# quinlan-lab/STRling

Measured on AMD Instinct MI355X. Metric: reads/sec through extract+cluster, 30x 150 bp WGS; 1/2/4/8 MI355X + CPU ref, higher is better.
Workload: dtype u8/u32 integer; 1 GPU; 1xMI355X: 30x 150 bp PE synthetic WGS, k=2-6 repeat-unit scorer + soft-clip scan + device pair logic + on-GPU radix-sort/segmented clustering (BASELINE.json configs[1]+[2]); reads_per_gpu=33554432, read_len=150, unique_reads_per_gpu=33554432, tiles=1, scored_reads=2843008, soft_items=993737, str_reads_clustered=514295, clusters=322142, bounds=5047, parallelism=records sharded over 1 GPU(s), no data-path collective

## Files before the change

### __graft_entry__.py

```python
import os
import sys

ROOT = os.path.dirname(os.path.abspath(__file__))
if ROOT not in sys.path:
    sys.path.insert(0, ROOT)


def build():
    import subprocess
    from strling_amd import build as b
    b.build(verbose=True)
    from oracle import oracle as O
    O.build()
    emu = os.path.join(ROOT, "tests", "emu")
    subprocess.check_call(["g++", "-O2", "-std=c++17", "-fPIC", "-shared", "-o", os.path.join(emu, "libscore_emu.so"),
                           os.path.join(emu, "score_emu.cpp")])
    subprocess.check_call(["g++", "-O2", "-std=c++17", "-fPIC", "-shared", "-o", os.path.join(emu, "libinflate_emu.so"),
                           os.path.join(emu, "inflate_emu.cpp")])
    import strling_amd
    from strling_amd import api, bamio
    bamio._bamgen()
    api.load(build_if_missing=False)


def smoke():
    import numpy as np
    from strling_amd import api, synth
    from oracle import oracle as O
    rec, g = synth.synth_wgs(4000, seed=42, contig_len=1_000_000)
    med = O.median(synth.frag_hist(rec))
    ctx = api.Context(0)
    ctx.set_opts(0.8, 40, med)
    ctx.set_genome(g)
    got, st = ctx.extract(rec)
    exp = O.extract(rec, g, O.make_opts(med, 0.8, 40))
    assert len(got) == len(exp) and len(exp) > 20, (len(got), len(exp))
    for f in ("tid", "position", "repeat", "flag", "split", "mapping_quality", "repeat_count", "align_length", "qname_id"):
        assert np.array_equal(got[f], exp[f]), f
    b, u, cs = ctx.cluster(got, api.MODE_CALL, 560, min_support=2, max_clip_dist=175)
    eb, eu = O.call_bounds(exp, 1, 560, min_support=2, max_clip_dist=175)
    assert [api.bounds_row(x, "c") for x in b] == [O.bounds_row(x, "c") for x in eb]
    assert "libstrling_amd.so" in open("/proc/self/maps").read()
    print(f"smoke ok: {rec.n} reads -> {len(got)} treads -> {len(b)} bounds; skipped {st.n_skipped}, scored {st.n_scored}, "
          f"soft items {st.n_soft_items}")
    ctx.close()


if __name__ == "__main__":
    build()
    if len(sys.argv) > 1 and sys.argv[1] == "smoke":
        smoke()
```

### strling_amd/csrc/score.hip

```cpp
#include <string.h>
#include <algorithm>
#include <thread>
#include <vector>
#include "common.h"
#include "host_score.h"
#include "device_util.h"
#include "score_core.h"
#include "score_tables.h"
#include "score.h"

namespace strl {

constexpr uint32_t EMPTY = 0xffffffffu;

struct ScoreParams {
  const uint4 *meta;
  uint64_t n;
  const int32_t *tid, *pos, *end;
  const uint32_t *seq_off;
  const uint16_t *l_seq, *clip_l, *clip_r;
  const uint8_t *mapq, *cig;
  const uint8_t *seq4;
  const TidInfo *g_tid;
  const int2 *g_iv;
// ... 150 lines not shown
      if (lane == 0) b = atomicAdd(&P.counters[CNT_QUEUE], cnt);
      b = __shfl(b, 0);
      __builtin_amdgcn_wave_barrier();
      for (uint32_t i = lane; i < cnt; i += 64) P.queue_id[b + i] = buf[i];
      __builtin_amdgcn_wave_barrier();
      cnt = 0;
    }
  };
  struct In { int4 t, s, e; uint32_t c; };
  constexpr int NIN = VEC ? CL_ILP / 4 : CL_ILP;
  auto load = [&](uint64_t base, In (&x)[NIN]) {
    if (VEC) {
#pragma unroll
      for (int gq = 0; gq < NIN; ++gq) {
        const uint64_t r = base + 256ull * gq + 4ull * lane;
        if (r + 3 < r1) {
          x[gq].t = reinterpret_cast<const int4 *>(P.tid)[r >> 2];
          x[gq].s = reinterpret_cast<const int4 *>(P.pos)[r >> 2];
          x[gq].e = reinterpret_cast<const int4 *>(P.end)[r >> 2];
          x[gq].c = reinterpret_cast<const uint32_t *>(P.cig)[r >> 2];
        } else {
          int32_t t[4], st[4], en[4];
          uint32_t cg = 0;
#pragma unroll
          for (int q = 0; q < 4; ++q) {
            const bool in = r + q < r1;
            cg |= (in ? (uint32_t)P.cig[r + q] : 0u) << (8 * q);
            t[q] = in ? P.tid[r + q] : -1; st[q] = in ? P.pos[r + q] : 0; en[q] = in ? P.end[r + q] : 0;
          }
          x[gq].t = make_int4(t[0], t[1], t[2], t[3]); x[gq].s = make_int4(st[0], st[1], st[2], st[3]);
          x[gq].e = make_int4(en[0], en[1], en[2], en[3]); x[gq].c = cg;
        }
      }
    } else {
#pragma unroll
      for (int j = 0; j < NIN; ++j) {
        const uint64_t r = base + 64 * j + lane;
        const bool in = r < r1;
        x[j].c = in ? P.cig[r] : 0u;
        x[j].t.x = in ? P.tid[r] : -1;
        x[j].s.x = in ? P.pos[r] : 0;
        x[j].e.x = in ? P.end[r] : 0;
      }
    }
  };
  auto comp = [](const int4 &v, int q) -> int32_t { return q == 0 ? v.x : q == 1 ? v.y : q == 2 ? v.z : v.w; };
  In cur[NIN], nxt[NIN];
  JoinState join;
  join.t = -2; join.valid = 0; join.lo = 0;
  load(r0, cur);
  for (uint64_t base = r0; base < r1; base += 64 * CL_ILP) {
    load(base + 64 * CL_ILP, nxt);
    bool need[CL_ILP], skipped[CL_ILP], inr[CL_ILP];
    uint32_t cgs[CL_ILP];
    int32_t ts[CL_ILP], sts[CL_ILP], ens[CL_ILP];
#pragma unroll
    for (int j = 0; j < CL_ILP; ++j) {
      inr[j] = ridx(base, j) < r1;
      if (VEC) {
        const In &g4 = cur[j >> 2];
        cgs[j] = (g4.c >> (8 * (j & 3))) & 0xffu; ts[j] = comp(g4.t, j & 3); sts[j] = comp(g4.s, j & 3); ens[j] = comp(g4.e, j & 3);
      } else {
        cgs[j] = cur[j].c; ts[j] = cur[j].t.x; sts[j] = cur[j].s.x; ens[j] = cur[j].e.x;
      }
    }
    skip_predicate_n<CL_ILP>(P, join, cgs, ts, sts, ens, inr, skipped);
#pragma unroll
    for (int j = 0; j < CL_ILP; ++j) {
      need[j] = inr[j] && !skipped[j];
      if (!VEC && skipped[j]) P.whole[ridx(base, j)] = STRL_RES_SKIPPED;
    }
    if (VEC) {
#pragma unroll
      for (int gq = 0; gq < CL_ILP / 4; ++gq) {
        const uint64_t r = base + 256ull * gq + 4ull * lane;
        if (r + 3 < r1) {
          reinterpret_cast<uint4 *>(P.whole)[r >> 2] = make_uint4(skipped[4 * gq] ? STRL_RES_SKIPPED : 0u, skipped[4 * gq + 1] ? STRL_RES_SKIPPED : 0u,
                                                                 skipped[4 * gq + 2] ? STRL_RES_SKIPPED : 0u, skipped[4 * gq + 3] ? STRL_RES_SKIPPED : 0u);
        } else {
#pragma unroll
          for (int q = 0; q < 4; ++q) if (skipped[4 * gq + q]) P.whole[r + q] = STRL_RES_SKIPPED;
        }
      }
    }
#pragma unroll
    for (int j = 0; j < CL_ILP; ++j) {
      const unsigned long long m = __ballot(need[j]);
      nskip += (uint32_t)__popcll(__ballot(skipped[j]));
      if (need[j]) buf[cnt + __popcll(m & below)] = (uint32_t)ridx(base, j);
      cnt += (uint32_t)__popcll(m);
    }
    if (cnt >= CL_STAGE) flush();
#pragma unroll
    for (int j = 0; j < NIN; ++j) cur[j] = nxt[j];
  }
  flush();
  if (lane == 0 && nskip) atomicAdd(&P.counters[CNT_SKIP], nskip);
}

template <int KIND, int MODE>
__global__ __launch_bounds__(1024) void compact_kernel(ScoreParams P) {
  __shared__ uint32_t wcnt[128];
  __shared__ uint32_t base_sh;
  const int lane = threadIdx.x & 63, wave = threadIdx.x >> 6;
  const unsigned long long below = (1ull << lane) - 1ull;
  uint32_t n_src, cap, cnt_idx;
  const uint4 *src;
  const uint4 *ent = nullptr;
  uint4 *dst;
  static_assert(KIND == 1, "soft items have their own compaction kernel");
  {
    n_src = MODE == 0 ? P.counters[CNT_QUEUE] : min(P.counters[CNT_SOFT], P.scap);
    src = P.sb_state[MODE]; ent = MODE == 0 ? P.queue : P.soft_queue; dst = P.sb_queue[MODE];
    cap = 0xffffffffu; cnt_idx = MODE == 0 ? CNT_SBW : CNT_SBS;
  }
  constexpr int U = 8;
  for (uint32_t b0 = blockIdx.x * (1024u * U); b0 < n_src; b0 += gridDim.x * (1024u * U)) {
    uint4 v[U];
    unsigned long long m[U];
#pragma unroll
    for (int u = 0; u < U; ++u) {
      const uint32_t i = b0 + 1024u * u + threadIdx.x;
      v[u] = make_uint4(EMPTY, 0, 0, 0);
      if (i < n_src) v[u] = src[i];
    }
#pragma unroll
    for (int u = 0; u < U; ++u) {
      m[u] = __ballot(v[u].x != EMPTY);
      if (lane == 0) wcnt[u * 16 + wave] = (uint32_t)__popcll(m[u]);
    }
    __syncthreads();
    if (threadIdx.x == 0) {
      uint32_t tot = 0;
      for (int w = 0; w < 16 * U; ++w) { const uint32_t c = wcnt[w]; wcnt[w] = tot; tot += c; }
      base_sh = tot ? atomicAdd(&P.counters[cnt_idx], tot) : 0u;
    }
    __syncthreads();
#pragma unroll
    for (int u = 0; u < U; ++u) {
      if (v[u].x != EMPTY) {
        const uint32_t i = b0 + 1024u * u + threadIdx.x;
        const uint32_t d = base_sh + wcnt[u * 16 + wave] + (uint32_t)__popcll(m[u] & below);
        if (KIND == 0) { if (d < cap) dst[d] = v[u]; }
        else {
          dst[2 * (uint64_t)d] = ent[i];
          dst[2 * (uint64_t)d + 1] = make_uint4(i, v[u].x, v[u].y, v[u].z);
        }
      }
    }
    __syncthreads();
  }
}

__global__ __launch_bounds__(1024) void soft_compact_kernel(ScoreParams P) {
  __shared__ uint32_t wcnt[128];
  __shared__ uint32_t base_sh;
  constexpr int U = 8;
  const int lane = threadIdx.x & 63, wave = threadIdx.x >> 6;
  const unsigned long long below = (1ull << lane) - 1ull;
  const uint32_t n_src = P.counters[CNT_QUEUE];
  for (uint32_t b0 = blockIdx.x * (1024u * U); b0 < n_src; b0 += gridDim.x * (1024u * U)) {
    uint32_t f[U];
    unsigned long long m0[U], m1[U];
#pragma unroll
    for (int u = 0; u < U; ++u) {
      const uint32_t i = b0 + 1024u * u + threadIdx.x;
      f[u] = i < n_src ? (uint32_t)P.soft_flag[i] : 0u;
    }
#pragma unroll
    for (int u = 0; u < U; ++u) {
      m0[u] = __ballot((f[u] & 1u) != 0);
      m1[u] = __ballot((f[u] & 2u) != 0);
      if (lane == 0) wcnt[u * 16 + wave] = (uint32_t)(__popcll(m0[u]) + __popcll(m1[u]));
    }
    __syncthreads();
    if (threadIdx.x == 0) {
      uint32_t tot = 0;
      for (int w = 0; w < 16 * U; ++w) { const uint32_t c = wcnt[w]; wcnt[w] = tot; tot += c; }
      base_sh = tot ? atomicAdd(&P.counters[CNT_SOFT], tot) : 0u;
    }
    __syncthreads();
#pragma unroll
    for (int u = 0; u < U; ++u) {
      if (f[u]) {
        const uint32_t i = b0 + 1024u * u + threadIdx.x;
        const uint4 e = P.queue[i];
        const uint32_t L = e.z & 0xffffu, cl = e.z >> 16, cr = e.w & 0xffffu;
        uint32_t d = base_sh + wcnt[u * 16 + wave] + (uint32_t)(__popcll(m0[u] & below) + __popcll(m1[u] & below));
        if (f[u] & 1u) { if (d < P.scap) P.soft_queue[d] = make_uint4(e.x << 1, e.y, 0u, cl < L ? cl : L); ++d; }
        if (f[u] & 2u) { const uint32_t c2 = cr < L ? cr : L; if (d < P.scap) P.soft_queue[d] = make_uint4((e.x << 1) | 1u, e.y, L - c2, c2); }
      }
    }
    __syncthreads();
  }
}

template <int NW, int SLOTS, int STAGE> constexpr int table_rows() {
  constexpr int raw = 4 * ((16 * NW + 62) / 32);
  constexpr int need = STAGE == 0 ? 24 : (NW <= 10 ? 0 : SLOTS);
  return raw > need ? raw : need;
}

__global__ void window_items_kernel(ScoreParams P, uint32_t n_win, uint32_t window, uint32_t step, uint64_t n_bases) {
  const uint32_t i = blockIdx.x * blockDim.x + threadIdx.x;
  if (i == 0) P.counters[CNT_SOFT] = n_win;
  if (i >= n_win) return;
  const uint64_t s0 = (uint64_t)i * step;
  const uint64_t len = s0 + window <= n_bases ? window : n_bases - s0;
  P.soft_queue[i] = make_uint4(i, 0u, (uint32_t)s0, (uint32_t)len);
}

__device__ inline uint32_t nt16_code(uint32_t ch) {
  switch (ch & ~0x20u) {
    case 'A': return 1; case 'C': return 2; case 'M': return 3; case 'G': return 4; case 'R': return 5; case 'S': return 6;
    case 'V': return 7; case 'T': return 8; case 'W': return 9; case 'Y': return 10; case 'H': return 11; case 'K': return 12;
    case 'D': return 13; case 'B': return 14; case 'N': return 15; default: return 0;
  }
}
__global__ __launch_bounds__(256) void pack_text_kernel(const uint8_t *__restrict__ text, uint32_t *__restrict__ seq4, uint64_t n_bases, uint64_t n_dwords) {
  __shared__ uint8_t tbl[256];
  tbl[threadIdx.x] = (uint8_t)nt16_code(threadIdx.x);
  __syncthreads();
  for (uint64_t d = (uint64_t)blockIdx.x * 256 + threadIdx.x; d < n_dwords; d += (uint64_t)gridDim.x * 256) {
    uint32_t out = 0;
    if (8 * d + 8 <= n_bases) {
      const uint2 t = *reinterpret_cast<const uint2 *>(text + 8 * d);
#pragma unroll
      for (int j = 0; j < 4; ++j) {
        const uint32_t w = j < 2 ? t.x >> (16 * j) : t.y >> (16 * (j - 2));
        out |= (((uint32_t)tbl[w & 0xffu] << 4) | tbl[(w >> 8) & 0xffu]) << (8 * j);
      }
    } else {
      for (int b = 0; b < 8; ++b) {
        const uint64_t i = 8 * d + b;
        const uint32_t cde = i < n_bases ? tbl[text[i]] : 0u;
        out |= cde << (8 * (b >> 1) + ((b & 1) ? 0 : 4));
      }
    }
    seq4[d] = out;
  }
}

template <int MODE, int STAGE> struct Item {
  uint32_t id, seq_off, slot;
  int L, len, s0;
  uint32_t cl, cr, cg, mq;
  int best;
  uint32_t res0, res1;
  bool act;
};

#ifndef STRL_SCORE_OCC
#define STRL_SCORE_OCC 5
#endif
template <int NW, int SLOTS, int MODE, int STAGE, int BLOCK>
__global__ __launch_bounds__(BLOCK, (BLOCK == 256 && NW <= 10) ? (STAGE == 0 ? STRL_SCORE_OCC : 4) : 1) void score_kernel(ScoreParams P) {
  constexpr int L56 = (LUT_ENTRIES - LUT_OFF5) / 2;
  constexpr int LUTK = STAGE == 0 ? LUT_A_DWORDS : STAGE == 1 ? LUT_DWORDS : LUT_A_DWORDS + L56;
  constexpr int LUTW = LUTK + 256;
  constexpr int NSLOT = STAGE == 2 ? INV_SLOTS / 2 : INV_SLOTS;
  constexpr int INV_AT = LUTW + (BLOCK / 64) * table_rows<NW, SLOTS, STAGE>() * 64;
  constexpr int LDS_WORDS = INV_AT + (BLOCK / 64) * NSLOT * NW;
  constexpr bool STATIC_LDS = (size_t)LDS_WORDS * 4 <= 65536;
  extern __shared__ __attribute__((aligned(16))) uint32_t lds_dyn[];
  __shared__ __attribute__((aligned(16))) uint32_t lds_st[STATIC_LDS ? LDS_WORDS : 4];
  uint32_t *const lds = STATIC_LDS ? lds_st : lds_dyn;
  if (STAGE == 2) {
    for (int i = threadIdx.x; i < LUT_A_DWORDS; i += BLOCK) lds[i] = P.ta[i];
    for (int i = threadIdx.x; i < L56; i += BLOCK) lds[LUT_A_DWORDS + i] = reinterpret_cast<const uint32_t *>(P.lut)[LUT_OFF5 / 2 + i];
  } else {
    for (int i = threadIdx.x; i < LUTK; i += BLOCK) lds[i] = STAGE == 0 ? P.ta[i] : reinterpret_cast<const uint32_t *>(P.lut)[i];
  }
  for (int i = threadIdx.x; i < 256; i += BLOCK) lds[LUTK + i] = reinterpret_cast<const uint32_t *>(P.lut)[LUT_DWORDS + i];
  __syncthreads();
  const uint16_t *lut = STAGE == 2 ? reinterpret_cast<const uint16_t *>(lds + LUT_A_DWORDS) - LUT_OFF5 : reinterpret_cast<const uint16_t *>(lds);
  const uint32_t *clut = lds + LUTK;
  const int lane = threadIdx.x & 63, wave = __builtin_amdgcn_readfirstlane(threadIdx.x >> 6);
  uint32_t *wave_tab = lds + LUTW + wave * (table_rows<NW, SLOTS, STAGE>() * 64);
  uint32_t *col = wave_tab + lane;
  constexpr int MAXCH = (16 * NW + 62) / 32;
  const int ROW0 = MODE == 0 ? 1 : P.seg_row0, ROW1 = MODE == 0 ? 1 : P.seg_row1;
  uint32_t n_items;
  const uint4 *q;
  if (STAGE == 1) { n_items = P.counters[MODE == 0 ? CNT_SBW : CNT_SBS]; q = P.sb_queue[MODE]; }
  else if (MODE == 0) { n_items = P.counters[CNT_QUEUE]; q = nullptr; }
  else { n_items = min(P.counters[CNT_SOFT], P.scap); q = P.soft_queue; }
  const uint32_t stride = gridDim.x * BLOCK;

  constexpr bool BY_ID = MODE == 0 && STAGE == 0;
  auto load_id = [&](uint32_t item) -> uint32_t { return (BY_ID && item < n_items) ? P.queue_id[item] : 0u; };
  struct Raw { uint4 e, x; };
  auto fetch = [&](uint32_t item, uint32_t rid) -> Raw {
    Raw r;
    r.e = make_uint4(0, 0, 0, 0);
    r.x = make_uint4(0, 0, 0, 0);
    if (BY_ID) {
      const uint4 m = P.meta[rid];
      r.e = make_uint4(rid, m.x, m.y, m.z);
      return r;
    }
    if (item < n_items) {
      if (BY_ID) { }
      else if (STAGE != 1) r.e = q[item];
      else { r.e = q[2 * (uint64_t)item]; r.x = q[2 * (uint64_t)item + 1]; }
    }
    return r;
  };
  auto unpack = [&](const Raw &r, uint32_t item) {
    Item<MODE, STAGE> it;
    const uint4 e = r.e, x = r.x;
    it.act = item < n_items;
    it.id = e.x; it.seq_off = e.y;
    it.L = (int)(e.z & 0xffffu);
    it.slot = STAGE != 1 ? item : x.x;
    it.best = STAGE != 1 ? -1 : (int)x.y;
    it.res0 = x.z; it.res1 = x.w;
    if (MODE == 0) {
      it.cl = e.z >> 16; it.cr = e.w & 0xffffu; it.cg = (e.w >> 16) & 0xffu; it.mq = e.w >> 24;
      if (it.L > STRL_DEVICE_READ_LEN) { it.L = 0; it.cl = 0; it.cr = 0; }
      it.len = it.L; it.s0 = 0;
    } else {
      it.cl = it.cr = it.cg = it.mq = 0;
      it.s0 = (int)e.z;
      it.len = (int)e.w;
      it.L = it.len;
    }
    if (it.len > 16 * NW) it.len = 16 * NW;
    if (!it.act) { it.len = 0; it.s0 = 0; }
    return it;
  };
  struct Pre { uint4 s[MAXCH]; LaneThr t; };
  auto prefetch = [&](const Item<MODE, STAGE> &it, Pre &p) {
    const int nch = it.act ? ((it.s0 & 31) + it.len + 31) >> 5 : 0;
    const uint4 *src = reinterpret_cast<const uint4 *>(P.seq4 + (uint64_t)it.seq_off * 16u) + (it.s0 >> 5);
#pragma unroll
    for (int c = 0; c < MAXCH; ++c) p.s[c] = (c < nch) ? src[c] : make_uint4(0, 0, 0, 0);
    load_thr(P.thr, ROW0, ROW1, it.len, p.t);
  };

  uint32_t base = blockIdx.x * BLOCK + wave * 64;
  Raw cur_r = fetch(base + lane, load_id(base + lane)), nxt_r = fetch(base + stride + lane, load_id(base + stride + lane));
  uint32_t id2 = load_id(base + 2 * stride + lane);
  Pre pc;
// ... 457 lines not shown
```

### strling_amd/csrc/score_core.h

```cpp
#pragma once
#include <stdint.h>

#ifdef STRL_EMU
#define STRL_DEV inline
#define STRL_HD inline
#define STRL_LANES 1
static inline uint32_t strl_funnel_r(uint32_t lo, uint32_t hi, uint32_t s) {
  return s == 0 ? lo : (uint32_t)(((((uint64_t)hi) << 32) | lo) >> s);
}
static inline int strl_ffs(uint32_t x) { return __builtin_ffs((int)x); }
static inline int strl_popc(uint32_t x) { return __builtin_popcount(x); }
static inline bool strl_any(bool p) { return p; }
static inline int strl_wave_min(int v) { return v; }
static inline uint32_t strl_max3(uint32_t a, uint32_t b, uint32_t c) { return a > b ? (a > c ? a : c) : (b > c ? b : c); }
static inline uint32_t strl_bfe(uint32_t x, uint32_t off, uint32_t w) { return (x >> off) & ((1u << w) - 1u); }
static inline uint32_t strl_lds_add(uint32_t *a, uint32_t v) { uint32_t o = *a; *a = o + v; return o; }
static inline int strl_wave_max(int v) { return v; }
static inline int strl_rank(bool) { return 0; }
static inline uint32_t strl_thread_at() { return 0; }
#else
#include <hip/hip_runtime.h>
#define STRL_DEV __device__ __forceinline__
#define STRL_HD __host__ __device__ __forceinline__
#define STRL_LANES 64
// ... 141 lines not shown
  static_assert(NRAW >= 2 * NW, "two raw dwords per word of the 2-bit stream");
  uint32_t any_f = 0, fl[NW];
#pragma unroll
  for (int h = 0; h < 2; ++h) {
    const int w0 = h ? NW / 2 : 0, w1 = h ? NW : NW / 2;
#pragma unroll
    for (int w = w0; w < w1; ++w) { sg.seq[w] = 0; fl[w] = 0; }
    if (h && 16 * w0 >= lb.hi) continue;
#pragma unroll
    for (int w = w0; w < w1; ++w) {
      const uint32_t a = conv_swizzle(raw[2 * w]), b = conv_swizzle(raw[2 * w + 1]);
      const uint32_t ra = clut[a & 0xffu] | (clut[(a >> 8) & 0xffu] << 4) | (clut[(a >> 16) & 0xffu] << 8) | (clut[a >> 24] << 12);
      const uint32_t rb = clut[b & 0xffu] | (clut[(b >> 8) & 0xffu] << 4) | (clut[(b >> 16) & 0xffu] << 8) | (clut[b >> 24] << 12);
      sg.seq[w] = (ra & 0xffffu) | (rb << 16);
      fl[w] = (ra >> 16) | (rb & 0xffff0000u);
    }
  }
#pragma unroll
  for (int w = 0; w < NW; ++w) {
    if (16 * (w + 1) > lb.lo) {
      const int nv = len - 16 * w;
      const uint32_t m = nv >= 16 ? 0xffffffffu : nv <= 0 ? 0u : ((1u << (2 * nv)) - 1u);
      sg.seq[w] &= m;
      fl[w] &= m;
    }
    any_f |= fl[w];
  }
  const int nn = inv_store<NW>(sg, any_f != 0, fl);
  sg.len = len;
  sg.n_N = nn;
}

template <int NW> STRL_DEV void seg_from_raw(const uint32_t *raw, const uint32_t *clut, int s0, int len, Seg<NW> &sg) {
  const int dw0 = s0 >> 3, sh = s0 & 7;
  uint32_t p, f;
  conv8_lut(raw[dw0 * STRL_LANES], clut, p, f);
  uint32_t cur = p >> (2 * sh), curf = f >> (2 * sh);
  const int fill = 16 - 2 * sh;
  uint32_t any_f = 0, fl[NW];
#pragma unroll
  for (int w = 0; w < NW; ++w) {
    uint32_t sw = 0, fw = 0;
    if (16 * w < len) {
      uint32_t pa, fa, pb, fb;
      conv8_lut(raw[(dw0 + 1 + 2 * w) * STRL_LANES], clut, pa, fa);
      conv8_lut(raw[(dw0 + 2 + 2 * w) * STRL_LANES], clut, pb, fb);
      uint64_t buf = (uint64_t)cur | ((uint64_t)pa << fill) | ((uint64_t)pb << (fill + 16));
      uint64_t bf = (uint64_t)curf | ((uint64_t)fa << fill) | ((uint64_t)fb << (fill + 16));
      sw = (uint32_t)buf;
      fw = (uint32_t)bf;
      cur = (uint32_t)(buf >> 32);
      curf = (uint32_t)(bf >> 32);
      const int nv = len - 16 * w;
      if (nv < 16) {
        const uint32_t m = (1u << (2 * nv)) - 1u;
        sw &= m;
        fw &= m;
      }
    }
    sg.seq[w] = sw;
    fl[w] = fw;
    any_f |= fw;
  }
  const int nn = inv_store<NW>(sg, any_f != 0, fl);
  sg.len = len;
  sg.n_N = nn;
}

template <int K, int NW> STRL_DEV uint32_t window_code(const Seg<NW> &sg, const uint16_t *lk, int i) {
  constexpr uint32_t MASK = (1u << (2 * K)) - 1u;
  const int bit = 2 * K * i, w = bit >> 5, sh = bit & 31;
  const uint32_t lo = sg.seq[w], hi = (w + 1 < NW) ? sg.seq[w + 1] : 0u;
  const uint32_t v = ((sh + 2 * K <= 32) ? (lo >> sh) : strl_funnel_r(lo, hi, sh)) & MASK;
  return lk[v];
}

template <int K, int NW>
STRL_DEV void hist_pass_a(const Seg<NW> &sg, bool active, uint32_t *bins0, uint32_t col_off, const uint32_t *ta, const LenBounds &lb, int &cmax, uint32_t &imax) {
  static_assert(K >= 2 && K <= 4, "stage A");
  constexpr uint32_t MASK = (1u << (2 * K)) - 1u;
  constexpr int NWIN = NW * 16 / K;
  constexpr int B = 8;
  constexpr int CS = K == 4 ? 24 : 19;
  constexpr uint32_t LOW = (1u << CS) - 1u;
  const int nwin = active ? sg.len / K : 0;
  const int umin = lb.lo == 0x7fffffff ? 0 : lb.lo / K, umax = lb.hi / K;
  const uint8_t *t3 = reinterpret_cast<const uint8_t *>(ta + TA_K3);
  cmax = 0;
  imax = MASK;
  uint32_t best = 0;
  auto kc = [](int j) { return (1u << CS) | ((7u - (uint32_t)j) << (CS - 3)); };
  auto entry = [&](int i) -> uint32_t {
    if (K == 2) return ta[TA_K2 + ((sg.seq[i >> 3] >> (8 * ((i >> 1) & 3))) & 0xffu)];
    if (K == 4) return ta[TA_K4 + ((sg.seq[i >> 2] >> (8 * (i & 3))) & 0xffu)];
    const int bit = 6 * i, w = bit >> 5, sh = bit & 31;
    const uint32_t lo = sg.seq[w], hi = (w + 1 < NW) ? sg.seq[w + 1] : 0u;
    return t3[((sh + 6 <= 32) ? (lo >> sh) : strl_funnel_r(lo, hi, sh)) & 63u];
  };
  auto entries = [&](int b0, uint32_t (&e)[B]) {
#pragma unroll
    for (int j = 0; j < B; ++j) e[j] = (b0 + j >= NWIN) ? 0u : (K == 2 && (j & 1)) ? e[j - 1] : entry(b0 + j);
  };
  auto count = [&](int j, uint32_t e) -> uint32_t {
    if (K == 4) {
      const uint32_t sh = (e >> 16) & 0xffu;
      uint32_t *bin = reinterpret_cast<uint32_t *>(reinterpret_cast<char *>(bins0) + (col_off + (e & 0xffffu)));
      const uint32_t old = strl_lds_add(bin, 1u << sh);
      return ((old >> sh) << 24) + (e + kc(j));
    }
    const uint32_t at = col_off + (K == 2 ? ((j & 1) ? (e >> 16) : (e & 0xffffu)) : e * ROWB);
    const uint32_t old = strl_lds_add(reinterpret_cast<uint32_t *>(reinterpret_cast<char *>(bins0) + at), 1u << CS);
    return old + kc(j) + at;
  };
  uint32_t e[B], en[B];
  entries(0, en);
#pragma unroll
  for (int b0 = 0; b0 < NWIN; b0 += B) {
#pragma unroll
    for (int j = 0; j < B; ++j) e[j] = en[j];
    if (b0 + B < NWIN) entries(b0 + B, en);
    if (b0 >= umax) continue;
    uint32_t key[B];
    if (b0 + B <= umin && b0 + B <= NWIN) {
#pragma unroll
      for (int j = 0; j < B; ++j) key[j] = count(j, e[j]);
    } else {
#pragma unroll
      for (int h = 0; h < B; h += B / 2) {
#pragma unroll
        for (int j = 0; j < B / 2; ++j) key[h + j] = 0;
        if (b0 + h < NWIN && b0 + h < umax) {
#pragma unroll
          for (int j = 0; j < B / 2; ++j)
            if (b0 + h + j < NWIN) {
              const uint32_t k = count(h + j, e[h + j]);
              key[h + j] = (b0 + h + j < nwin) ? k : 0u;
            }
        }
      }
    }
    uint32_t bb = key[0] > key[1] ? key[0] : key[1];
#pragma unroll
    for (int j = 2; j + 1 < B; j += 2) bb = strl_max3(bb, key[j], key[j + 1]);
    if (bb > (best | LOW)) best = bb;
  }
  if (best) {
    const uint16_t *tc = reinterpret_cast<const uint16_t *>(ta + TA_C) + TaCls<K>::off;
    cmax = (int)(best >> CS);
    if (K == 4) imax = tc[4u * ((best & 0xffffu) / ROWB) + ((best >> 19) & 3u)];
    else imax = tc[((best & 0xffffu) - col_off) / ROWB];
  }
}

template <int K, int NW, int SLOTS>
STRL_DEV void hist_pass(const Seg<NW> &sg, bool active, uint32_t *tab, const uint16_t *lut, int &cmax, uint32_t &imax) {
  static_assert(K >= 5, "stage B");
  constexpr uint32_t MASK = (1u << (2 * K)) - 1u;
  constexpr int NWIN = NW * 16 / K;
  constexpr int B = 8;
  const uint16_t *lk = lut + LutOff<K>::v;
  const int nwin = active ? sg.len / K : 0;
  cmax = 0;
  imax = MASK;
  if (NW <= 10) {
    uint32_t code[NWIN];
#pragma unroll
    for (int i = 0; i < NWIN; ++i) code[i] = window_code<K, NW>(sg, lk, i);
#pragma unroll
    for (int i = 0; i < NWIN; ++i) {
      uint32_t ne = 0;
#pragma unroll
      for (int j = 0; j < i; ++j) {
        const uint32_t x = code[j] ^ code[i];
        ne += x < 1u ? x : 1u;
      }
      const int newc = 1 + i - (int)ne;
      if (i < nwin && newc > cmax) { cmax = newc; imax = code[i]; }
    }
    return;
  }
#pragma unroll
  for (int b0 = 0; b0 < NWIN; b0 += B) {
    if (!strl_any(b0 < nwin)) break;
    uint32_t code[B];
#pragma unroll
    for (int j = 0; j < B; ++j) code[j] = (b0 + j < NWIN) ? window_code<K, NW>(sg, lk, b0 + j) : 0u;
    {
#pragma unroll
      for (int j = 0; j < B; ++j) {
        if (b0 + j < NWIN && b0 + j < nwin) {
          const uint32_t c = code[j];
          uint32_t hsh = ((c * 0x9E3779B1u) >> 16) & (uint32_t)(SLOTS - 1);
          int newc;
          for (;;) {
            const uint32_t e = tab[hsh * STRL_LANES];
            if (e == 0) { tab[hsh * STRL_LANES] = ((c + 1u) << 8) | 1u; newc = 1; break; }
            if ((e >> 8) == c + 1u) { tab[hsh * STRL_LANES] = e + 1u; newc = (int)(e & 0xffu) + 1; break; }
            hsh = (hsh + 1u) & (uint32_t)(SLOTS - 1);
          }
          if (newc > cmax) { cmax = newc; imax = c; }
        }
      }
    }
  }
}

template <int K, int NW> STRL_DEV int recount(const Seg<NW> &sg, uint32_t code, int lo_len) {
  uint32_t acc[NW];
#pragma unroll
  for (int w = 0; w < NW; ++w) acc[w] = 0;
  uint32_t iv[NW];
  if (sg.has_inv()) inv_load<NW>(sg, iv);
#pragma unroll
  for (int j = 0; j < K; ++j) {
    const uint32_t pat = ((code >> (2 * (K - 1 - j))) & 3u) * 0x55555555u;
#pragma unroll
    for (int w = 0; w < NW; ++w) {
      const uint32_t lo = sg.seq[w], hi = (w + 1 < NW) ? sg.seq[w + 1] : 0u;
      acc[w] |= strl_funnel_r(lo, hi, 2 * j) ^ pat;
    }
  }
  if (sg.has_inv()) {
#pragma unroll
    for (int j = 0; j < K; ++j) {
#pragma unroll
      for (int w = 0; w < NW; ++w) {
        const uint32_t lo = iv[w], hi = (w + 1 < NW) ? iv[w + 1] : 0u;
        acc[w] |= strl_funnel_r(lo, hi, 2 * j);
      }
    }
  }
  const int limit = sg.len - K + 1;
  uint32_t m[NW];
#pragma unroll
  for (int w = 0; w < NW; ++w) {
    uint32_t x = ~(acc[w] | (acc[w] >> 1)) & 0x55555555u;
    if (16 * (w + 1) > lo_len - K + 1) {
      const int nv = limit - 16 * w;
      if (nv < 16) x &= (nv <= 0) ? 0u : ((1u << (2 * nv)) - 1u);
    }
    m[w] = x;
  }
  int cnt = 0;
  if (K == 2) {
    uint32_t carry = 0;
#pragma unroll
    for (int w = 0; w < NW; ++w) {
      const uint32_t prev = w ? m[w - 1] : 0u;
      const uint32_t start = m[w] & ~((m[w] << 2) | (prev >> 30));
      const uint32_t fill = m[w] | (m[w] << 1);
      const uint64_t t = (uint64_t)fill + (start & 0x11111111u) + carry;
      carry = (uint32_t)(t >> 32);
      const uint32_t even_runs = fill & ~(uint32_t)t;
      const uint32_t sel = (m[w] & even_runs & 0x11111111u) | (m[w] & ~even_runs & 0x44444444u);
      cnt += strl_popc(sel);
    }
  } else {
    bool border = false;
#pragma unroll
    for (int d = 1; d < K; ++d) border |= (code >> (2 * d)) == (code & ((1u << (2 * (K - d))) - 1u));
    if (!strl_any(border)) {
#pragma unroll
      for (int w = 0; w < NW; ++w) cnt += strl_popc(m[w]);
    } else {
      int skip = 0;
#pragma unroll
      for (int w = 0; w < NW; ++w) {
        uint32_t x = m[w] & ~((1u << (2 * skip)) - 1u);
        skip = 0;
        while (x) {
          const int i = (strl_ffs(x) - 1) >> 1;
          ++cnt;
          const int nx = i + K;
          if (nx >= 16) { skip = nx - 16; x = 0; }
          else x &= ~((1u << (2 * nx)) - 1u);
        }
      }
    }
  }
  return cnt;
}

STRL_DEV void clear_rows(uint32_t *wave_tab, int lane, int rows) {
#ifdef STRL_EMU
  for (int i = 0; i < rows; ++i) wave_tab[i] = 0;
  (void)lane;
#else
  uint4 z = make_uint4(0, 0, 0, 0);
  uint4 *p = reinterpret_cast<uint4 *>(wave_tab);
  const int n16 = rows * (STRL_LANES / 4);
  __builtin_amdgcn_wave_barrier();
  for (int i = lane; i < n16; i += STRL_LANES) p[i] = z;
  __builtin_amdgcn_wave_barrier();
#endif
}

struct ScoreState {
  int best;
  bool alive;
  uint32_t res0, res1;
  unsigned long long ph_t;
};

template <int K, int SLOTS> struct KRows { static constexpr int v = (K == 2) ? 10 : (K == 3) ? 24 : (K == 4) ? 18 : SLOTS; };

struct LaneThr {
  uint64_t w12, w0, w1;
};
STRL_DEV void load_thr(const uint64_t *thr, int row0, int row1, int L, LaneThr &t) {
  t.w12 = thr[0 * THR_LMAX + L];
  t.w0 = thr[row0 * THR_LMAX + L];
  t.w1 = (row1 == row0) ? t.w0 : thr[row1 * THR_LMAX + L];
}
template <int K> STRL_DEV int thr_get(uint64_t w) { return (int)((w >> (8 * (K - 2))) & 0xffu); }

template <int K, int NW, int SLOTS>
STRL_DEV void score_k(const Seg<NW> &sg, ScoreState &st, uint32_t *wave_tab, int lane, const void *tables, const LaneThr &t, const LenBounds &lb, uint32_t *bins0) {
  if (!strl_any(st.alive)) return;
  if (K <= 4 || NW > 10) clear_rows(wave_tab, lane, KRows<K, SLOTS>::v);
  int c;
  uint32_t code;
  if constexpr (K <= 4) hist_pass_a<K, NW>(sg, st.alive, bins0, (uint32_t)((wave_tab - bins0) + lane) * 4u, static_cast<const uint32_t *>(tables), lb, c, code);
  else hist_pass<K, NW, SLOTS>(sg, st.alive, wave_tab + lane, static_cast<const uint16_t *>(tables), c, code);
  STRL_PH(st, 2 + 2 * (K - 2));
  if (st.alive) {
    int score = c * K;
    if (score <= st.best) {
      if (c < thr_get<K>(t.w12)) st.alive = false;
    } else {
#if defined(STRL_PHASE_TIMING) && !defined(STRL_EMU)
      {
        const unsigned long long bm = __ballot(true);
        if ((threadIdx.x & 63) == (unsigned)(__ffsll((long long)bm) - 1)) { atomicAdd(&g_phase[23 + 2 * (K - 2) - (K > 4 ? 4 : 0)], 1ull); atomicAdd(&g_phase[24 + 2 * (K - 2) - (K > 4 ? 4 : 0)], (unsigned long long)__popcll(bm)); }
      }
#endif
#ifdef STRL_EXP_SKIP_RECOUNT34
      if (K != 3 && K != 4)
#endif
      c = recount<K, NW>(sg, code, lb.lo == 0x7fffffff ? 0 : lb.lo);
      score = c * K;
      if (score >= st.best) {
        st.best = score;
        const uint32_t packed = code | ((uint32_t)K << 12) | ((uint32_t)c << 16);
        if (c > thr_get<K>(t.w0)) st.res0 = packed;
        if (c > thr_get<K>(t.w1)) st.res1 = packed;
      }
    }
  }
  STRL_PH(st, 3 + 2 * (K - 2));
}

STRL_DEV uint32_t reduce_packed(uint32_t r) {
  const uint32_t k = (r >> 12) & 7u;
  if (k == 0) return 0;
  const uint32_t code = r & 0xfffu, b = code & 3u;
  const uint32_t rep = b * (((1u << (2 * k)) - 1u) / 3u);
  if (code != rep) return r;
  return b | (1u << 12) | (((r >> 16) * k) << 16);
}

template <int NW, int SLOTS>
STRL_DEV void score_stage_a(const Seg<NW> &sg, bool active, uint32_t *wave_tab, uint32_t *bins0, int lane, const uint32_t *ta, const LaneThr &t,
                            const LenBounds &lb, ScoreState &st) {
  st.best = -1;
  st.alive = active && sg.n_N <= 20;
  st.res0 = st.res1 = 0;
  score_k<2, NW, SLOTS>(sg, st, wave_tab, lane, ta, t, lb, bins0);
  score_k<3, NW, SLOTS>(sg, st, wave_tab, lane, ta, t, lb, bins0);
  score_k<4, NW, SLOTS>(sg, st, wave_tab, lane, ta, t, lb, bins0);
}
template <int NW, int SLOTS>
STRL_DEV void score_stage_b(const Seg<NW> &sg, uint32_t *wave_tab, int lane, const uint16_t *lut, const LaneThr &t, const LenBounds &lb, ScoreState &st) {
  score_k<5, NW, SLOTS>(sg, st, wave_tab, lane, lut, t, lb, nullptr);
  score_k<6, NW, SLOTS>(sg, st, wave_tab, lane, lut, t, lb, nullptr);
}

}
```

Measured before the change: 29.19 billion reads/s.

## Bound K5/6 histogram and recount by wave length, bin soft-clip queue by length

The k=5/6 histogram now runs in blocks of four windows and stops once past the wave's maximum segment length (lb.hi/K). The recount is restructured to go word by word and stop past hi_len, which avoids work on padding words. Soft-clip compaction now groups output entries by clip-length class within each block, so downstream consumers see more uniform work per wave. This costs extra LDS atomics and holds all queue entries in registers.

```diff
diff --git a/__graft_entry__.py b/__graft_entry__.py
--- a/__graft_entry__.py
+++ b/__graft_entry__.py
@@ -15,6 +15,8 @@
     emu = os.path.join(ROOT, "tests", "emu")
     subprocess.check_call(["g++", "-O2", "-std=c++17", "-fPIC", "-shared", "-o", os.path.join(emu, "libscore_emu.so"),
                            os.path.join(emu, "score_emu.cpp")])
+    subprocess.check_call(["g++", "-O2", "-std=c++17", "-fPIC", "-shared", "-o", os.path.join(emu, "libscore_bounds_emu.so"),
+                           os.path.join(emu, "score_bounds_emu.cpp")])
     subprocess.check_call(["g++", "-O2", "-std=c++17", "-fPIC", "-shared", "-o", os.path.join(emu, "libinflate_emu.so"),
                            os.path.join(emu, "inflate_emu.cpp")])
     import strling_amd
diff --git a/strling_amd/csrc/score.hip b/strling_amd/csrc/score.hip
--- a/strling_amd/csrc/score.hip
+++ b/strling_amd/csrc/score.hip
@@ -326,20 +326,30 @@
   }
 }
 
+constexpr int SOFT_NCLS = 22;
+__device__ __forceinline__ uint32_t soft_len_class(uint32_t len) { return len <= 160u ? (len + 7u) >> 3 : (uint32_t)SOFT_NCLS - 1u; }
 __global__ __launch_bounds__(1024) void soft_compact_kernel(ScoreParams P) {
   __shared__ uint32_t wcnt[128];
-  __shared__ uint32_t base_sh;
+  __shared__ uint32_t ccnt[SOFT_NCLS];
+  __shared__ uint32_t base_sh, tot_sh;
   constexpr int U = 8;
   const int lane = threadIdx.x & 63, wave = threadIdx.x >> 6;
   const unsigned long long below = (1ull << lane) - 1ull;
   const uint32_t n_src = P.counters[CNT_QUEUE];
   for (uint32_t b0 = blockIdx.x * (1024u * U); b0 < n_src; b0 += gridDim.x * (1024u * U)) {
-    uint32_t f[U];
+    uint32_t f[U], rank[U];
+    uint4 e[U];
     unsigned long long m0[U], m1[U];
+    if (threadIdx.x < SOFT_NCLS) ccnt[threadIdx.x] = 0;
 #pragma unroll
     for (int u = 0; u < U; ++u) {
       const uint32_t i = b0 + 1024u * u + threadIdx.x;
       f[u] = i < n_src ? (uint32_t)P.soft_flag[i] : 0u;
+    }
+#pragma unroll
+    for (int u = 0; u < U; ++u) {
+      e[u] = make_uint4(0, 0, 0, 0);
+      if (f[u]) e[u] = P.queue[b0 + 1024u * u + threadIdx.x];
     }
 #pragma unroll
     for (int u = 0; u < U; ++u) {
@@ -348,21 +358,39 @@
       if (lane == 0) wcnt[u * 16 + wave] = (uint32_t)(__popcll(m0[u]) + __popcll(m1[u]));
     }
     __syncthreads();
+#pragma unroll
+    for (int u = 0; u < U; ++u) {
+      const uint32_t L = e[u].z & 0xffffu, cl = min(e[u].z >> 16, L), cr = min(e[u].w & 0xffffu, L);
+      rank[u] = 0;
+      if (f[u] & 1u) rank[u] = atomicAdd(&ccnt[soft_len_class(cl)], 1u);
+      if (f[u] & 2u) rank[u] |= atomicAdd(&ccnt[soft_len_class(cr)], 1u) << 16;
+    }
+    __syncthreads();
     if (threadIdx.x == 0) {
       uint32_t tot = 0;
       for (int w = 0; w < 16 * U; ++w) { const uint32_t c = wcnt[w]; wcnt[w] = tot; tot += c; }
+      uint32_t at = 0;
+      for (int c = 0; c < SOFT_NCLS; ++c) { const uint32_t k = ccnt[c]; ccnt[c] = at; at += k; }
       base_sh = tot ? atomicAdd(&P.counters[CNT_SOFT], tot) : 0u;
+      tot_sh = tot;
     }
     __syncthreads();
+    const uint32_t base = base_sh;
+    const bool binned = (uint64_t)base + tot_sh <= P.scap;
 #pragma unroll
     for (int u = 0; u < U; ++u) {
       if (f[u]) {
-        const uint32_t i = b0 + 1024u * u + threadIdx.x;
-        const uint4 e = P.queue[i];
-        const uint32_t L = e.z & 0xffffu, cl = e.z >> 16, cr = e.w & 0xffffu;
-        uint32_t d = base_sh + wcnt[u * 16 + wave] + (uint32_t)(__popcll(m0[u] & below) + __popcll(m1[u] & below));
-        if (f[u] & 1u) { if (d < P.scap) P.soft_queue[d] = make_uint4(e.x << 1, e.y, 0u, cl < L ? cl : L); ++d; }
-        if (f[u] & 2u) { const uint32_t c2 = cr < L ? cr : L; if (d < P.scap) P.soft_queue[d] = make_uint4((e.x << 1) | 1u, e.y, L - c2, c2); }
+        const uint32_t L = e[u].z & 0xffffu, cl = min(e[u].z >> 16, L), cr = min(e[u].w & 0xffffu, L);
+        uint32_t d = base + wcnt[u * 16 + wave] + (uint32_t)(__popcll(m0[u] & below) + __popcll(m1[u] & below));
+        if (f[u] & 1u) {
+          const uint32_t at = binned ? base + ccnt[soft_len_class(cl)] + (rank[u] & 0xffffu) : d;
+          if (at < P.scap) P.soft_queue[at] = make_uint4(e[u].x << 1, e[u].y, 0u, cl);
+          ++d;
+        }
+        if (f[u] & 2u) {
+          const uint32_t at = binned ? base + ccnt[soft_len_class(cr)] + (rank[u] >> 16) : d;
+          if (at < P.scap) P.soft_queue[at] = make_uint4((e[u].x << 1) | 1u, e[u].y, L - cr, cr);
+        }
       }
     }
     __syncthreads();
diff --git a/strling_amd/csrc/score_core.h b/strling_amd/csrc/score_core.h
--- a/strling_amd/csrc/score_core.h
+++ b/strling_amd/csrc/score_core.h
@@ -317,8 +317,32 @@
   }
 }
 
+constexpr int HB56 = 4;
+template <int K, int NW, int B0>
+STRL_DEV void hist56_blocks(const Seg<NW> &sg, const uint16_t *lk, int nwin, int umax, uint32_t (&code)[NW * 16 / K], int &cmax, uint32_t &imax) {
+  constexpr int NWIN = NW * 16 / K;
+  if constexpr (B0 < NWIN) {
+    if (B0 >= umax) return;
+    constexpr int B1 = B0 + HB56 < NWIN ? B0 + HB56 : NWIN;
+#pragma unroll
+    for (int i = B0; i < B1; ++i) code[i] = window_code<K, NW>(sg, lk, i);
+#pragma unroll
+    for (int i = B0; i < B1; ++i) {
+      uint32_t ne = 0;
+#pragma unroll
+      for (int j = 0; j < i; ++j) {
+        const uint32_t x = code[j] ^ code[i];
+        ne += x < 1u ? x : 1u;
+      }
+      const int newc = 1 + i - (int)ne;
+      if (i < nwin && newc > cmax) { cmax = newc; imax = code[i]; }
+    }
+    hist56_blocks<K, NW, B1>(sg, lk, nwin, umax, code, cmax, imax);
+  }
+}
+
 template <int K, int NW, int SLOTS>
-STRL_DEV void hist_pass(const Seg<NW> &sg, bool active, uint32_t *tab, const uint16_t *lut, int &cmax, uint32_t &imax) {
+STRL_DEV void hist_pass(const Seg<NW> &sg, bool active, uint32_t *tab, const uint16_t *lut, const LenBounds &lb, int &cmax, uint32_t &imax) {
   static_assert(K >= 5, "stage B");
   constexpr uint32_t MASK = (1u << (2 * K)) - 1u;
   constexpr int NWIN = NW * 16 / K;
@@ -327,21 +351,9 @@
   const int nwin = active ? sg.len / K : 0;
   cmax = 0;
   imax = MASK;
-  if (NW <= 10) {
+  if constexpr (NW <= 10) {
     uint32_t code[NWIN];
-#pragma unroll
-    for (int i = 0; i < NWIN; ++i) code[i] = window_code<K, NW>(sg, lk, i);
-#pragma unroll
-    for (int i = 0; i < NWIN; ++i) {
-      uint32_t ne = 0;
-#pragma unroll
-      for (int j = 0; j < i; ++j) {
-        const uint32_t x = code[j] ^ code[i];
-        ne += x < 1u ? x : 1u;
-      }
-      const int newc = 1 + i - (int)ne;
-      if (i < nwin && newc > cmax) { cmax = newc; imax = code[i]; }
-    }
+    hist56_blocks<K, NW, 0>(sg, lk, nwin, lb.hi / K, code, cmax, imax);
     return;
   }
 #pragma unroll
@@ -370,80 +382,66 @@
   }
 }
 
-template <int K, int NW> STRL_DEV int recount(const Seg<NW> &sg, uint32_t code, int lo_len) {
-  uint32_t acc[NW];
-#pragma unroll
-  for (int w = 0; w < NW; ++w) acc[w] = 0;
+struct RecountRun { uint32_t prev, carry; int skip, cnt; };
+template <int K, int NW, int W>
+STRL_DEV void recount_words(const Seg<NW> &sg, const uint32_t (&pat)[K], const uint32_t (&iv)[NW], bool walk, int lo_len, int hi_len, RecountRun &r) {
+  if constexpr (W < NW) {
+    if (16 * W >= hi_len) return;
+    const uint32_t lo = sg.seq[W], hi = (W + 1 < NW) ? sg.seq[W + 1] : 0u;
+    uint32_t acc = 0;
+#pragma unroll
+    for (int j = 0; j < K; ++j) acc |= strl_funnel_r(lo, hi, 2 * j) ^ pat[j];
+    if (sg.has_inv()) {
+      const uint32_t ilo = iv[W], ihi = (W + 1 < NW) ? iv[W + 1] : 0u;
+#pragma unroll
+      for (int j = 0; j < K; ++j) acc |= strl_funnel_r(ilo, ihi, 2 * j);
+    }
+    uint32_t m = ~(acc | (acc >> 1)) & 0x55555555u;
+    if (16 * (W + 1) > lo_len - K + 1) {
+      const int nv = sg.len - K + 1 - 16 * W;
+      if (nv < 16) m &= (nv <= 0) ? 0u : ((1u << (2 * nv)) - 1u);
+    }
+    if (K == 2) {
+      const uint32_t start = m & ~((m << 2) | (r.prev >> 30));
+      const uint32_t fill = m | (m << 1);
+      const uint64_t t = (uint64_t)fill + (start & 0x11111111u) + r.carry;
+      r.carry = (uint32_t)(t >> 32);
+      const uint32_t even_runs = fill & ~(uint32_t)t;
+      const uint32_t sel = (m & even_runs & 0x11111111u) | (m & ~even_runs & 0x44444444u);
+      r.cnt += strl_popc(sel);
+      r.prev = m;
+    } else if (!walk) {
+      r.cnt += strl_popc(m);
+    } else {
+      uint32_t x = m & ~((1u << (2 * r.skip)) - 1u);
+      r.skip = 0;
+      while (x) {
+        const int i = (strl_ffs(x) - 1) >> 1;
+        ++r.cnt;
+        const int nx = i + K;
+        if (nx >= 16) { r.skip = nx - 16; x = 0; }
+        else x &= ~((1u << (2 * nx)) - 1u);
+      }
+    }
+    recount_words<K, NW, W + 1>(sg, pat, iv, walk, lo_len, hi_len, r);
+  }
+}
+
+template <int K, int NW> STRL_DEV int recount(const Seg<NW> &sg, uint32_t code, int lo_len, int hi_len) {
   uint32_t iv[NW];
   if (sg.has_inv()) inv_load<NW>(sg, iv);
-#pragma unroll
-  for (int j = 0; j < K; ++j) {
-    const uint32_t pat = ((code >> (2 * (K - 1 - j))) & 3u) * 0x55555555u;
-#pragma unroll
-    for (int w = 0; w < NW; ++w) {
-      const uint32_t lo = sg.seq[w], hi = (w + 1 < NW) ? sg.seq[w + 1] : 0u;
-      acc[w] |= strl_funnel_r(lo, hi, 2 * j) ^ pat;
-    }
-  }
-  if (sg.has_inv()) {
-#pragma unroll
-    for (int j = 0; j < K; ++j) {
-#pragma unroll
-      for (int w = 0; w < NW; ++w) {
-        const uint32_t lo = iv[w], hi = (w + 1 < NW) ? iv[w + 1] : 0u;
-        acc[w] |= strl_funnel_r(lo, hi, 2 * j);
-      }
-    }
-  }
-  const int limit = sg.len - K + 1;
-  uint32_t m[NW];
-#pragma unroll
-  for (int w = 0; w < NW; ++w) {
-    uint32_t x = ~(acc[w] | (acc[w] >> 1)) & 0x55555555u;
-    if (16 * (w + 1) > lo_len - K + 1) {
-      const int nv = limit - 16 * w;
-      if (nv < 16) x &= (nv <= 0) ? 0u : ((1u << (2 * nv)) - 1u);
-    }
-    m[w] = x;
-  }
-  int cnt = 0;
-  if (K == 2) {
-    uint32_t carry = 0;
-#pragma unroll
-    for (int w = 0; w < NW; ++w) {
-      const uint32_t prev = w ? m[w - 1] : 0u;
-      const uint32_t start = m[w] & ~((m[w] << 2) | (prev >> 30));
-      const uint32_t fill = m[w] | (m[w] << 1);
-      const uint64_t t = (uint64_t)fill + (start & 0x11111111u) + carry;
-      carry = (uint32_t)(t >> 32);
-      const uint32_t even_runs = fill & ~(uint32_t)t;
-      const uint32_t sel = (m[w] & even_runs & 0x11111111u) | (m[w] & ~even_runs & 0x44444444u);
-      cnt += strl_popc(sel);
-    }
-  } else {
-    bool border = false;
+  uint32_t pat[K];
+#pragma unroll
+  for (int j = 0; j < K; ++j) pat[j] = ((code >> (2 * (K - 1 - j))) & 3u) * 0x55555555u;
+  bool border = false;
+  if (K > 2) {
 #pragma unroll
     for (int d = 1; d < K; ++d) border |= (code >> (2 * d)) == (code & ((1u << (2 * (K - d))) - 1u));
-    if (!strl_any(border)) {
-#pragma unroll
-      for (int w = 0; w < NW; ++w) cnt += strl_popc(m[w]);
-    } else {
-      int skip = 0;
-#pragma unroll
-      for (int w = 0; w < NW; ++w) {
-        uint32_t x = m[w] & ~((1u << (2 * skip)) - 1u);
-        skip = 0;
-        while (x) {
-          const int i = (strl_ffs(x) - 1) >> 1;
-          ++cnt;
-          const int nx = i + K;
-          if (nx >= 16) { skip = nx - 16; x = 0; }
-          else x &= ~((1u << (2 * nx)) - 1u);
-        }
-      }
-    }
-  }
-  return cnt;
+  }
+  const bool walk = K > 2 && strl_any(border);
+  RecountRun r = {0u, 0u, 0, 0};
+  recount_words<K, NW, 0>(sg, pat, iv, walk, lo_len, hi_len, r);
+  return r.cnt;
 }
 
 STRL_DEV void clear_rows(uint32_t *wave_tab, int lane, int rows) {
@@ -486,7 +484,7 @@
   int c;
   uint32_t code;
   if constexpr (K <= 4) hist_pass_a<K, NW>(sg, st.alive, bins0, (uint32_t)((wave_tab - bins0) + lane) * 4u, static_cast<const uint32_t *>(tables), lb, c, code);
-  else hist_pass<K, NW, SLOTS>(sg, st.alive, wave_tab + lane, static_cast<const uint16_t *>(tables), c, code);
+  else hist_pass<K, NW, SLOTS>(sg, st.alive, wave_tab + lane, static_cast<const uint16_t *>(tables), lb, c, code);
   STRL_PH(st, 2 + 2 * (K - 2));
   if (st.alive) {
     int score = c * K;
@@ -502,7 +500,7 @@
 #ifdef STRL_EXP_SKIP_RECOUNT34
       if (K != 3 && K != 4)
 #endif
-      c = recount<K, NW>(sg, code, lb.lo == 0x7fffffff ? 0 : lb.lo);
+      c = recount<K, NW>(sg, code, lb.lo == 0x7fffffff ? 0 : lb.lo, lb.hi);
       score = c * K;
       if (score >= st.best) {
         st.best = score;
```

After: 30.43 billion reads/s (median of 6 runs). 4.2% higher.
